# buaacyw/GaussianEditor

Hardware: AMD Instinct MI355X
Metric: train iters/sec (fwd+bwd of one 1080p view per GPU + grad all-reduce), 1M Gaussians @1080p (higher is better)
Workload: dtype f32; 1 GPU; synth-v1 1000000 Gaussians SH3 (M=16, s0=0.01), 1920x1080, ring-v1 8 views, one view per GPU (BASELINE.json configs[3] shape; configs[1] bicycle.ply is not available offline); gaussians=1000000, width=1920, height=1080, views_per_rank=1, parallelism=dp1-views, view_pipeline=False, tile_bounds=reference, fast_exp=False, grad_exchange=direct, grad_exchange_route=local, grad_rows=every row of every gradient written every iteration, num_rendered=0, visible=0, pixel_instances=0, sort_key_bits=45

## Files before the change

gaussianeditor_amd/csrc/gsr_binning.hip:

```cpp
#include <stdlib.h>

#include "gsr_kernels.h"

namespace gsr {

__device__ __forceinline__ int f2i_sat(float v) {
  if (!(v == v)) return 0;
  if (v >= 2147483648.0f) return 2147483647;
  if (v <= -2147483648.0f) return (-2147483647 - 1);
  return (int)v;
}

constexpr int RBITS = 8;
constexpr int RBINS = 1 << RBITS;

template <class K, int TH, bool WEIGHTED = false>
__global__ void __launch_bounds__(TH) sort_hist_kernel(const K* __restrict__ keys, int64_t n, int shift,
                                                                uint32_t mask, uint32_t* __restrict__ hist,
                                                                uint32_t nblocks, const uint4* __restrict__ publish_src,
                                                                uint32_t publish_count, uint32_t* __restrict__ publish_dst,
                                                                uint32_t publish_seq, const uint32_t* __restrict__ rect32) {
  __shared__ uint32_t h[RBINS];
  __shared__ uint32_t hw[WEIGHTED ? RBINS : 1];
  if (publish_dst != nullptr && blockIdx.x == nblocks) {
// ... 597 lines not shown
    constexpr int NV = (int)(sizeof(K) * RANGE_PER / sizeof(uint4));
    const uint4* __restrict__ src = reinterpret_cast<const uint4*>(tkeys + base);
    uint4 v[NV];
#pragma unroll
    for (int i = 0; i < NV; ++i) v[i] = src[i];
    __builtin_memcpy(k, v, sizeof(k));
  } else {
#pragma unroll
    for (int i = 0; i < RANGE_PER; ++i) k[i] = base + i < L ? tkeys[base + i] : (K)0;
  }
  uint32_t prev = base ? (uint32_t)tkeys[base - 1] : 0u;
#pragma unroll
  for (int i = 0; i < RANGE_PER; ++i) {
    const int64_t idx = base + i;
    if (idx >= L) break;
    const uint32_t cur = (uint32_t)k[i];
    if (idx == 0) {
      ranges[cur].x = 0;
    } else if (cur != prev) {
      ranges[prev].y = (uint32_t)idx;
      ranges[cur].x = (uint32_t)idx;
    }
    if (idx == L - 1) ranges[cur].y = (uint32_t)L;
    prev = cur;
  }
}

__global__ void __launch_bounds__(1024) tile_worklist_kernel(int T, uint2* __restrict__ ranges,
                                                            uint32_t* __restrict__ order, uint32_t* __restrict__ meta,
                                                            uint32_t* __restrict__ queues, uint32_t* __restrict__ est,
                                                            const uint32_t* __restrict__ tile_total,
                                                            uint32_t* __restrict__ tile_start, uint32_t* __restrict__ ck_table,
                                                            uint32_t n_ck_tiles) {
  constexpr int WORK_SUB = 16, NCNT = (WORK_BUCKETS + 1) * WORK_SUB, WORK_LDS_TILES = 8192;
  __shared__ uint32_t cnt[NCNT];
  __shared__ uint32_t smem[1024 / 64 + 1];
  __shared__ uint32_t s_len[WORK_LDS_TILES];
  const bool cached = T <= WORK_LDS_TILES;
  const bool split = gridDim.x == 2;
  const bool do_prefix = tile_total != nullptr && (!split || blockIdx.x == 0);
  const bool do_sort = !split || blockIdx.x == 1;
  for (int i = threadIdx.x; i < NCNT; i += 1024) cnt[i] = 0;
  if (do_prefix) {
    constexpr int PER = 8;
    uint32_t carry = 0;
    for (int base = 0; base < T; base += 1024 * PER) {
      const int i0 = base + (int)threadIdx.x * PER;
      const bool full = i0 + PER <= T;
      uint32_t v[PER], sum = 0;
      if (full) {
        const uint4 a0 = reinterpret_cast<const uint4*>(tile_total + i0)[0], a1 = reinterpret_cast<const uint4*>(tile_total + i0)[1];
        v[0] = a0.x; v[1] = a0.y; v[2] = a0.z; v[3] = a0.w; v[4] = a1.x; v[5] = a1.y; v[6] = a1.z; v[7] = a1.w;
      } else {
#pragma unroll
        for (int j = 0; j < PER; ++j) v[j] = i0 + j < T ? tile_total[i0 + j] : 0u;
      }
#pragma unroll
      for (int j = 0; j < PER; ++j) sum += v[j];
      uint32_t chunk;
      uint32_t run = carry + block_excl_scan_u32<1024>(sum, &chunk, smem);
      uint32_t st[PER];
#pragma unroll
      for (int j = 0; j < PER; ++j) {
        st[j] = run;
        run += v[j];
      }
      if (full) {
        reinterpret_cast<uint4*>(tile_start + i0)[0] = make_uint4(st[0], st[1], st[2], st[3]);
        reinterpret_cast<uint4*>(tile_start + i0)[1] = make_uint4(st[4], st[5], st[6], st[7]);
#pragma unroll
        for (int j = 0; j < PER; j += 2)
          reinterpret_cast<uint4*>(ranges + i0)[j / 2] = make_uint4(v[j] ? st[j] : 0u, v[j] ? st[j] + v[j] : 0u,
                                                                   v[j + 1] ? st[j + 1] : 0u, v[j + 1] ? st[j + 1] + v[j + 1] : 0u);
      }
#pragma unroll
      for (int j = 0; j < PER; ++j) {
        if (i0 + j < T) {
          if (!full) {
            tile_start[i0 + j] = st[j];
            ranges[i0 + j] = v[j] ? make_uint2(st[j], st[j] + v[j]) : make_uint2(0u, 0u);
          }
          if (cached) s_len[i0 + j] = v[j];
        }
      }
      carry += chunk;
    }
    if (threadIdx.x == 0) tile_start[T] = carry;
  } else if (cached && tile_total != nullptr) {
    for (int t = threadIdx.x; t < T; t += 1024) s_len[t] = tile_total[t];
  } else if (cached) {
    for (int t = threadIdx.x; t < T; t += 1024) {
      const uint2 r = ranges[t];
      s_len[t] = r.y - r.x;
    }
  }
  if (!do_sort) return;
  __syncthreads();
  auto len_of = [&](int t) -> uint32_t {
    if (cached) return s_len[t];
    if (tile_total != nullptr) return tile_total[t];
    const uint2 r = ranges[t];
    return r.y - r.x;
  };
  const uint32_t sub = threadIdx.x & (WORK_SUB - 1);
  auto bucket_of = [](uint32_t len) -> uint32_t {
    if (len == 0) return WORK_BUCKETS;
    const uint32_t c = (len + 63u) / 64u;
    return (uint32_t)(WORK_BUCKETS - 1) - min(c - 1u, (uint32_t)(WORK_BUCKETS - 1));
  };
  for (int t = threadIdx.x; t < T; t += 1024) atomicAdd(&cnt[bucket_of(len_of(t)) * WORK_SUB + sub], 1u);
  __syncthreads();
  {
    constexpr int CPT = (NCNT + 1023) / 1024;
    const int i0 = (int)threadIdx.x * CPT;
    uint32_t v[CPT], sum = 0;
#pragma unroll
    for (int j = 0; j < CPT; ++j) {
      v[j] = i0 + j < NCNT ? cnt[i0 + j] : 0u;
      sum += v[j];
    }
    uint32_t all;
    uint32_t run = block_excl_scan_u32<1024>(sum, &all, smem);
#pragma unroll
    for (int j = 0; j < CPT; ++j) {
      if (i0 + j < NCNT) cnt[i0 + j] = run;
      if (i0 + j == WORK_BUCKETS * WORK_SUB) meta[0] = run;
      run += v[j];
    }
  }
  __syncthreads();
  for (int t = threadIdx.x; t < T; t += 1024) {
    const uint32_t len = len_of(t);
    const uint32_t pos = atomicAdd(&cnt[bucket_of(len) * WORK_SUB + sub], 1u);
    order[pos] = (uint32_t)t;
    ck_table[t] = (len != 0u && pos < n_ck_tiles) ? pos : CK_NONE;
  }
  for (int i = threadIdx.x; i < 8 * T; i += 1024) est[i] = 0u;
  for (int i = threadIdx.x; i < QUEUE_KINDS * QUEUE_LINES; i += 1024) {
    queues[(size_t)i * QUEUE_STRIDE] = 0u;
    queues[(size_t)i * QUEUE_STRIDE + 1] = 0u;
  }
}

template <int BITS, int TH>
__global__ void __launch_bounds__(TH) group_hist_kernel(const uint32_t* __restrict__ keys, int64_t n,
                                                                 uint32_t* __restrict__ hist, uint32_t nblocks,
                                                                 uint32_t* __restrict__ fill_dst, int64_t fill_n) {
  constexpr int NB = 1 << BITS;
  __shared__ uint32_t h[NB];
  for (int i = threadIdx.x; i < NB; i += TH) h[i] = 0;
  (void)fill_dst;
  (void)fill_n;
  __syncthreads();
  const int64_t base = (int64_t)blockIdx.x * SORT_KPB;
  uint32_t kv[(SORT_KPB / TH)];
#pragma unroll
  for (int i = 0; i < (SORT_KPB / TH); ++i) {
    const int64_t k = base + (int64_t)i * TH + threadIdx.x;
    kv[i] = (uint32_t)keys[k < n ? k : n - 1];
  }
#pragma unroll
  for (int i = 0; i < (SORT_KPB / TH); ++i) {
    const int64_t k = base + (int64_t)i * TH + threadIdx.x;
    if (k < n) atomicAdd(&h[kv[i] & (NB - 1)], 1u);
  }
  __syncthreads();
  for (int i = threadIdx.x; i < NB; i += TH) hist[(size_t)i * nblocks + blockIdx.x] = h[i];
}

template <int BITS, int TH>
__global__ void __launch_bounds__(TH) group_scatter_kernel(const uint32_t* __restrict__ keys_in,
                                                                    const uint32_t* __restrict__ vals_in,
                                                                    uint32_t* __restrict__ keys_out,
                                                                    uint32_t* __restrict__ vals_out, int64_t n,
                                                                    const uint32_t* __restrict__ hist,
                                                                    const uint32_t* __restrict__ bin_total,
                                                                    uint32_t nblocks, uint32_t chunk,
                                                                    uint32_t* __restrict__ group_first) {
  constexpr int NB = 1 << BITS, NW = TH / 64, ITEMS = SORT_KPB / TH;
  constexpr int BT = NB < TH ? NB : TH, BPT = NB / BT;
  const bool owns = (int)threadIdx.x < BT;
  __shared__ uint16_t cnt[NW][NB];
  __shared__ uint32_t gbase[NB];
  __shared__ uint16_t lexcl[NB];
  __shared__ uint32_t smem[TH / 64 + 1];
  __shared__ uint32_t skey[SORT_KPB];
  __shared__ uint32_t sval[SORT_KPB];
  const int w = (int)(threadIdx.x >> 6), l = lane_id();
  const int64_t bbase = (int64_t)blockIdx.x * SORT_KPB;
  const int64_t wbase = bbase + (int64_t)w * (ITEMS * 64);
  uint32_t key[ITEMS], val[ITEMS];
  uint16_t rank[ITEMS];
  const uint64_t lt_mask = (1ull << l) - 1ull;
#pragma unroll
  for (int i = 0; i < ITEMS; ++i) {
    const int64_t k = wbase + (int64_t)i * 64 + l;
    const int64_t kc = k < n ? k : n - 1;
    key[i] = keys_in[kc];
    val[i] = vals_in[kc];
  }
  {
    uint32_t padded[BPT], mine[BPT], sum = 0;
#pragma unroll
    for (int j = 0; j < BPT; ++j) {
      const uint32_t d = owns ? threadIdx.x * BPT + j : 0u;
      const uint32_t tot = owns ? bin_total[d] : 0u;
      padded[j] = (tot + chunk - 1u) / chunk * chunk;
      mine[j] = owns ? hist[(size_t)d * nblocks + blockIdx.x] : 0u;
      sum += padded[j];
    }
    uint32_t tot;
    uint32_t run = block_excl_scan_u32<TH>(sum, &tot, smem);
    if (owns) {
#pragma unroll
      for (int j = 0; j < BPT; ++j) {
        gbase[threadIdx.x * BPT + j] = run + mine[j];
        if (blockIdx.x == 0) group_first[threadIdx.x * BPT + j] = run / chunk;
        run += padded[j];
      }
      if (blockIdx.x == 0 && (int)threadIdx.x == BT - 1) group_first[NB] = run / chunk;
    }
  }
  for (int i = threadIdx.x; i < NW * NB; i += TH) (&cnt[0][0])[i] = 0;
  __syncthreads();

#pragma unroll
  for (int i = 0; i < ITEMS; ++i) {
    const int64_t k = wbase + (int64_t)i * 64 + l;
    const bool valid = k < n;
    const uint32_t d = key[i] & (NB - 1);
    uint64_t m = __ballot(valid);
#pragma unroll
    for (int b = 0; b < BITS; ++b) {
      const uint64_t bb = __ballot((d >> b) & 1u);
      m &= ((d >> b) & 1u) ? bb : ~bb;
    }
    const uint32_t before = (uint32_t)__popcll(m & lt_mask);
    uint32_t old = 0;
    if (valid) old = cnt[w][d];
    if (valid && before == 0) cnt[w][d] = (uint16_t)(old + (uint32_t)__popcll(m));
    rank[i] = (uint16_t)(old + before);
  }
  __syncthreads();
  {
    uint32_t tot_d[BPT], sum = 0;
#pragma unroll
    for (int j = 0; j < BPT; ++j) {
      const uint32_t d = owns ? threadIdx.x * BPT + j : 0u;
      uint32_t run = 0;
      if (owns) {
#pragma unroll
        for (int i = 0; i < NW; ++i) {
          const uint32_t c = cnt[i][d];
          cnt[i][d] = (uint16_t)run;
          run += c;
        }
      }
      tot_d[j] = run;
      sum += run;
    }
    uint32_t tot;
    uint32_t run = block_excl_scan_u32<TH>(sum, &tot, smem);
    if (owns) {
#pragma unroll
      for (int j = 0; j < BPT; ++j) {
        lexcl[threadIdx.x * BPT + j] = (uint16_t)run;
        run += tot_d[j];
      }
    }
  }
  __syncthreads();
#pragma unroll
  for (int i = 0; i < ITEMS; ++i) {
    const int64_t k = wbase + (int64_t)i * 64 + l;
    if (k < n) {
      const uint32_t d = key[i] & (NB - 1);
      const uint32_t lp = (uint32_t)lexcl[d] + (uint32_t)cnt[w][d] + rank[i];
      skey[lp] = key[i];
      sval[lp] = val[i];
    }
  }
  __syncthreads();
  const int nvalid = (int)min((int64_t)SORT_KPB, n - bbase);
#pragma unroll
  for (int i = 0; i < ITEMS; ++i) {
    const int j = i * TH + (int)threadIdx.x;
    if (j < nvalid) {
      const uint32_t kk = skey[j], d = kk & (NB - 1);
      const uint32_t pos = gbase[d] + ((uint32_t)j - (uint32_t)lexcl[d]);
      keys_out[pos] = kk;
      vals_out[pos] = sval[j];
    }
  }
}

struct GroupArgs {
  int gx, gy, sgx;
  size_t chunks;
  uint32_t stage_cap;
  const uint32_t* gkey;
  const uint32_t* gval;
  uint16_t* chunk_cnt;
  const uint32_t* chunk_pre;
  const uint32_t* tile_start;
  uint32_t* point_list;
};

__device__ __forceinline__ void group_mask(uint32_t lr, uint32_t& lo, uint32_t& hi) {
  const uint32_t x0 = lr & 7u, x1 = (lr >> 3) & 7u, y0 = (lr >> 6) & 7u, y1 = (lr >> 9) & 7u;
  const uint32_t cols = ((2u << (x1 - x0)) - 1u) << x0;
  const uint64_t rows = ((~0ull >> (56u - 8u * (y1 - y0))) << (8u * y0)) & 0x0101010101010101ull;
  lo = (uint32_t)rows * cols;
  hi = (uint32_t)(rows >> 32) * cols;
}

struct TransposeLane {
  uint32_t keep[5], rot[5];
};
__device__ __forceinline__ TransposeLane transpose_lane_consts(int lane) {
  constexpr uint32_t LOW[5] = {0x0000ffffu, 0x00ff00ffu, 0x0f0f0f0fu, 0x33333333u, 0x55555555u};
  TransposeLane c;
#pragma unroll
  for (int i = 0; i < 5; ++i) {
    const int d = 16 >> i;
    const bool up = (lane & d) != 0;
    c.keep[i] = up ? ~LOW[i] : LOW[i];
    c.rot[i] = up ? (uint32_t)d : (uint32_t)(32 - d);
  }
  return c;
}
template <int STAGE>
__device__ __forceinline__ uint32_t transpose_partner(uint32_t x) {
  const int v = (int)x;
  if constexpr (STAGE == 0) return (uint32_t)__builtin_amdgcn_ds_swizzle(v, 0x401f);
  else if constexpr (STAGE == 1) return (uint32_t)__builtin_amdgcn_update_dpp(0, v, 0x128, 0xf, 0xf, false);
  else if constexpr (STAGE == 2) return (uint32_t)__builtin_amdgcn_ds_swizzle(v, 0x101f);
  else if constexpr (STAGE == 3) return (uint32_t)__builtin_amdgcn_update_dpp(0, v, 0x4e, 0xf, 0xf, false);
  else return (uint32_t)__builtin_amdgcn_update_dpp(0, v, 0xb1, 0xf, 0xf, false);
}
template <int STAGE>
__device__ __forceinline__ void transpose_stage(const TransposeLane& c, uint32_t& lo, uint32_t& hi) {
  const uint32_t pl = transpose_partner<STAGE>(lo), ph = transpose_partner<STAGE>(hi);
  const uint32_t rl = __builtin_amdgcn_alignbit(pl, pl, c.rot[STAGE]), rh = __builtin_amdgcn_alignbit(ph, ph, c.rot[STAGE]);
  lo = (c.keep[STAGE] & lo) | (~c.keep[STAGE] & rl);
  hi = (c.keep[STAGE] & hi) | (~c.keep[STAGE] & rh);
}
__device__ __forceinline__ void transpose_masks(const TransposeLane& c, uint32_t lo, uint32_t hi, uint32_t& wlo, uint32_t& whi) {
  {
    const auto r = __builtin_amdgcn_permlane32_swap(lo, hi, false, false);
    lo = r[0];
    hi = r[1];
  }
  transpose_stage<0>(c, lo, hi);
  transpose_stage<1>(c, lo, hi);
  transpose_stage<2>(c, lo, hi);
  transpose_stage<3>(c, lo, hi);
  transpose_stage<4>(c, lo, hi);
  wlo = lo;
  whi = hi;
}

template <bool SCATTER, int NB>
__global__ void __launch_bounds__(64) group_chunk_kernel(const GroupArgs a) {
  extern __shared__ __align__(8) unsigned char stage_raw[];
  uint2* const stage = reinterpret_cast<uint2*>(stage_raw);
  const size_t c = (size_t)(blockIdx.x & 7u) * (gridDim.x >> 3) + (blockIdx.x >> 3);
  if (c >= a.chunks) return;
  const int lane = (int)threadIdx.x;
  const size_t base = c * (size_t)(64 * NB);
  uint32_t key[NB], idx[NB];
#pragma unroll
  for (int b = 0; b < NB; ++b) {
    key[b] = a.gkey[base + (size_t)b * 64 + lane];
    idx[b] = SCATTER ? a.gval[base + (size_t)b * 64 + lane] : 0u;
  }
  const uint32_t first = (uint32_t)__builtin_amdgcn_readfirstlane((int)key[0]);
  if (first == GROUP_PAD) return;
  const TransposeLane tc = transpose_lane_consts(lane);
  const uint32_t cap = a.stage_cap;
  uint32_t cnt = 0, g = 0, staged = 0;
  if (SCATTER) {
    const uint32_t s = first & 0xffffu;
    const uint32_t tx = ((s % (uint32_t)a.sgx) << GROUP_SHIFT) + (uint32_t)(lane & 7);
    const uint32_t ty = ((s / (uint32_t)a.sgx) << GROUP_SHIFT) + (uint32_t)(lane >> 3);
    const bool tile_ok = tx < (uint32_t)a.gx && ty < (uint32_t)a.gy;
    g = tile_ok ? a.tile_start[ty * (uint32_t)a.gx + tx] + a.chunk_pre[c * GROUP_TILES + lane] : 0u;
  }
  auto flush = [&]() {
    __syncthreads();
    for (uint32_t e = (uint32_t)lane; e < staged; e += 64u) {
      const uint2 x = stage[e];
      a.point_list[x.y] = x.x;
    }
    __syncthreads();
    staged = 0;
  };
#pragma unroll
  for (int b = 0; b < NB; ++b) {
    const bool valid = key[b] != GROUP_PAD;
    if (b > 0 && __ballot(valid) == 0ull) break;
    uint32_t lo = 0u, hi = 0u;
    if (valid) group_mask(key[b] >> 16, lo, hi);
    uint32_t wlo, whi;
    transpose_masks(tc, lo, hi, wlo, whi);
    if (!SCATTER) {
      cnt += (uint32_t)__popc(wlo) + (uint32_t)__popc(whi);
    } else {
      const uint32_t nl = (uint32_t)__popc(wlo), nh = (uint32_t)__popc(whi);
      const uint32_t tot_l = (uint32_t)__builtin_amdgcn_readlane((int)wave_incl_scan_dpp(nl), 63);
      const uint32_t tot_h = (uint32_t)__builtin_amdgcn_readlane((int)wave_incl_scan_dpp(nh), 63);
      const int nparts = tot_l + tot_h <= cap ? 1 : (max(tot_l, tot_h) <= cap ? 2 : 4);
      for (int part = 0; part < nparts; ++part) {
        uint32_t wa = wlo, wb = whi;
        if (nparts == 2) {
          wa = part == 0 ? wlo : 0u;
          wb = part == 0 ? 0u : whi;
        } else if (nparts == 4) {
          const uint32_t m = 0xffffu << (16 * (part & 1));
          wa = part < 2 ? (wlo & m) : 0u;
          wb = part < 2 ? 0u : (whi & m);
        }
        const uint32_t na = (uint32_t)__popc(wa), np = na + (uint32_t)__popc(wb);
        const uint32_t incl = wave_incl_scan_dpp(np);
        const uint32_t total = (uint32_t)__builtin_amdgcn_readlane((int)incl, 63);
        if (staged + total > cap) flush();
        uint32_t curA = staged + incl - np, curB = curA + na, gA = g, gB = g + na;
        while (__ballot((wa | wb) != 0u) != 0ull) {
          const bool va = wa != 0u, vb = wb != 0u;
          const int ja = va ? __builtin_ctz(wa) : 0, jb = vb ? 32 + __builtin_ctz(wb) : 0;
          const uint32_t xa = (uint32_t)__shfl((int)idx[b], ja, 64), xb = (uint32_t)__shfl((int)idx[b], jb, 64);
          stage[va ? curA : cap] = make_uint2(xa, gA);
          stage[vb ? curB : cap] = make_uint2(xb, gB);
          curA += va ? 1u : 0u;
          gA += va ? 1u : 0u;
          curB += vb ? 1u : 0u;
          gB += vb ? 1u : 0u;
          wa &= wa - 1u;
          wb &= wb - 1u;
        }
        staged += total;
        g += np;
      }
    }
  }
  if (SCATTER) flush();
  if (!SCATTER) a.chunk_cnt[c * GROUP_TILES + lane] = (uint16_t)cnt;
}

constexpr int COLSCAN_WAVES = 16, COLSCAN_REG = 16;
__global__ void __launch_bounds__(COLSCAN_WAVES * 64) group_colscan_kernel(int gx, int gy, int sgx,
                                                                          const uint32_t* __restrict__ group_first,
                                                                          const uint16_t* __restrict__ chunk_cnt,
                                                                          uint32_t* __restrict__ chunk_pre,
                                                                          uint32_t* __restrict__ tile_total) {
  __shared__ uint32_t slab[COLSCAN_WAVES][GROUP_TILES];
  const uint32_t s = blockIdx.x;
  const int w = (int)(threadIdx.x >> 6), lane = lane_id();
  const uint32_t first = group_first[s], n = group_first[s + 1] - first;
  const uint32_t per = (n + COLSCAN_WAVES - 1) / COLSCAN_WAVES;
  const uint32_t r0 = min(n, (uint32_t)w * per), r1 = min(n, r0 + per);
  const uint16_t* __restrict__ src = chunk_cnt + (size_t)(first + r0) * GROUP_TILES + lane;
  uint32_t* __restrict__ out = chunk_pre + (size_t)(first + r0) * GROUP_TILES + lane;
  const uint32_t rows = r1 - r0;
  auto load_rows = [&](uint32_t first_row, uint32_t (&v)[COLSCAN_REG]) {
    const uint32_t last = rows - 1u;
    uint32_t raw[COLSCAN_REG];
#pragma unroll
    for (int i = 0; i < COLSCAN_REG; ++i) raw[i] = (uint32_t)src[(size_t)min(first_row + (uint32_t)i, last) * GROUP_TILES];
#pragma unroll
    for (int i = 0; i < COLSCAN_REG; ++i) v[i] = first_row + (uint32_t)i < rows ? raw[i] : 0u;
  };
  uint32_t v0[COLSCAN_REG];
  uint32_t sum = 0;
#pragma unroll
  for (int i = 0; i < COLSCAN_REG; ++i) v0[i] = 0u;
  if (rows != 0u) {
    load_rows(0u, v0);
#pragma unroll
    for (int i = 0; i < COLSCAN_REG; ++i) sum += v0[i];
    for (uint32_t r = COLSCAN_REG; r < rows; r += COLSCAN_REG) {
      uint32_t v[COLSCAN_REG];
      load_rows(r, v);
#pragma unroll
      for (int i = 0; i < COLSCAN_REG; ++i) sum += v[i];
    }
  }
  slab[w][lane] = sum;
  __syncthreads();
  uint32_t run = 0, total = 0;
#pragma unroll
  for (int i = 0; i < COLSCAN_WAVES; ++i) {
    const uint32_t x = slab[i][lane];
    run += i < w ? x : 0u;
    total += x;
  }
#pragma unroll
  for (int i = 0; i < COLSCAN_REG; ++i) {
    if ((uint32_t)i < rows) out[(size_t)i * GROUP_TILES] = run;
    run += v0[i];
  }
  for (uint32_t r = COLSCAN_REG; r < rows; r += COLSCAN_REG) {
    uint32_t v[COLSCAN_REG];
    load_rows(r, v);
#pragma unroll
    for (int i = 0; i < COLSCAN_REG; ++i) {
      if (r + (uint32_t)i < rows) out[(size_t)(r + (uint32_t)i) * GROUP_TILES] = run;
      run += v[i];
    }
  }
  if (w == 0) {
    const uint32_t tx = ((s % (uint32_t)sgx) << GROUP_SHIFT) + (uint32_t)(lane & 7);
    const uint32_t ty = ((s / (uint32_t)sgx) << GROUP_SHIFT) + (uint32_t)(lane >> 3);
    if (tx < (uint32_t)gx && ty < (uint32_t)gy) tile_total[ty * (uint32_t)gx + tx] = total;
  }
}

template <bool SCATTER>
static void launch_chunks(hipStream_t s, const Binning& b, const GroupArgs& a) {
  const dim3 grid((unsigned)((b.chunks + 7) / 8 * 8)), block(64);
  const size_t lds = SCATTER ? sizeof(uint2) * ((size_t)a.stage_cap + 1) : 0;
  switch (b.chunk / 64) {
    case 1: hipLaunchKernelGGL((group_chunk_kernel<SCATTER, 1>), grid, block, lds, s, a); break;
    case 2: hipLaunchKernelGGL((group_chunk_kernel<SCATTER, 2>), grid, block, lds, s, a); break;
    case 4: hipLaunchKernelGGL((group_chunk_kernel<SCATTER, 4>), grid, block, lds, s, a); break;
    default: hipLaunchKernelGGL((group_chunk_kernel<SCATTER, 8>), grid, block, lds, s, a); break;
  }
}

static int64_t checkpoint_state_words(const Image& im);
template <int BITS>
static void launch_grouped(hipStream_t s, int P, int64_t R, int gx, int gy, const Geom& g, const Binning& b, const Image& im) {
  const int nbg = (P + GAUSS_BLOCK - 1) / GAUSS_BLOCK;
  const int64_t padded = b.chunks * (int64_t)b.chunk;
  const int fill_blocks = 512;
  hipLaunchKernelGGL(emit_groups_kernel, dim3(nbg + fill_blocks), dim3(GAUSS_BLOCK), 0, s, P, b.sgx, g, b.gkey[0], b.gval[0], nbg,
                     b.gkey[1], padded, reinterpret_cast<uint4*>(im.ck_work), checkpoint_state_words(im) / 4);
  const bool wide = b.sort_blocks <= SORT_WIDE_MAX_BLOCKS;
  if (wide)
    hipLaunchKernelGGL((group_hist_kernel<BITS, 1024>), dim3(b.sort_blocks), dim3(1024), 0, s, (const uint32_t*)b.gkey[0], b.G,
                       b.ghist, b.sort_blocks, b.gkey[1], padded);
  else
    hipLaunchKernelGGL((group_hist_kernel<BITS, SORT_THREADS>), dim3(b.sort_blocks), dim3(SORT_THREADS), 0, s,
                       (const uint32_t*)b.gkey[0], b.G, b.ghist, b.sort_blocks, b.gkey[1], padded);
  hipLaunchKernelGGL(sort_scan_kernel, dim3(1 << BITS), dim3(SORT_THREADS), 0, s, b.ghist, b.gbin_total, b.sort_blocks);
  if (wide)
    hipLaunchKernelGGL((group_scatter_kernel<BITS, 1024>), dim3(b.sort_blocks), dim3(1024), 0, s, (const uint32_t*)b.gkey[0],
                       (const uint32_t*)b.gval[0], b.gkey[1], b.gval[1], b.G, (const uint32_t*)b.ghist,
                       (const uint32_t*)b.gbin_total, b.sort_blocks, (uint32_t)b.chunk, b.group_first);
  else
    hipLaunchKernelGGL((group_scatter_kernel<BITS, SORT_THREADS>), dim3(b.sort_blocks), dim3(SORT_THREADS), 0, s,
                       (const uint32_t*)b.gkey[0], (const uint32_t*)b.gval[0], b.gkey[1], b.gval[1], b.G, (const uint32_t*)b.ghist,
                       (const uint32_t*)b.gbin_total, b.sort_blocks, (uint32_t)b.chunk, b.group_first);
  GroupArgs a;
  a.gx = gx; a.gy = gy; a.sgx = b.sgx; a.chunks = (size_t)b.chunks;
  a.stage_cap = (R / b.G + 1) * (int64_t)b.chunk <= 820 ? 1024u : 2048u;
  a.gkey = b.gkey[1]; a.gval = b.gval[1];
  a.chunk_cnt = b.chunk_cnt; a.chunk_pre = b.chunk_pre; a.tile_start = b.tile_start; a.point_list = b.point_list;
  launch_chunks<false>(s, b, a);
  hipLaunchKernelGGL(group_colscan_kernel, dim3(b.groups), dim3(COLSCAN_WAVES * 64), 0, s, gx, gy, b.sgx,
                     (const uint32_t*)b.group_first, (const uint16_t*)b.chunk_cnt, b.chunk_pre, b.tile_total);
  hipLaunchKernelGGL(tile_worklist_kernel, dim3(2), dim3(1024), 0, s, gx * gy, im.ranges, im.work_order, im.work_meta,
                     im.queue_heads, im.work_est, (const uint32_t*)b.tile_total, b.tile_start, im.ck_table,
                     (uint32_t)ck_tiles((size_t)gx * gy));
  launch_chunks<true>(s, b, a);
}

static int64_t checkpoint_state_words(const Image& im) {
  return (int64_t)((reinterpret_cast<const char*>(im.ck_pool) - reinterpret_cast<const char*>(im.ck_work)) / 4);
}

hipError_t launch_binning(hipStream_t s, int P, int64_t R, int W, int H, const Geom& g, const Binning& b, const Image& im) {
  const int gx = (W + TILE - 1) / TILE, gy = (H + TILE - 1) / TILE;
  if (R <= 0 || b.legacy) {
    hipError_t e = hipMemsetAsync(im.ck_work, 0, sizeof(uint32_t) * (size_t)checkpoint_state_words(im), s);
    if (e != hipSuccess) return e;
  }
  if (R <= 0) {
    hipError_t e = hipMemsetAsync(im.ranges, 0, sizeof(uint2) * (size_t)gx * gy, s);
    if (e != hipSuccess) return e;
    hipLaunchKernelGGL(tile_worklist_kernel, dim3(1), dim3(1024), 0, s, gx * gy, im.ranges, im.work_order, im.work_meta,
                       im.queue_heads, im.work_est, (const uint32_t*)nullptr, (uint32_t*)nullptr, im.ck_table,
                       (uint32_t)ck_tiles((size_t)gx * gy));
    return hipGetLastError();
  }
  if (!b.legacy) {
    if (b.group_bits == 8) launch_grouped<8>(s, P, R, gx, gy, g, b, im);
    else launch_grouped<11>(s, P, R, gx, gy, g, b, im);
    return hipGetLastError();
  }
  const int nbg = (P + GAUSS_BLOCK - 1) / GAUSS_BLOCK;
  const dim3 ge(max(nbg, (gx * gy + GAUSS_BLOCK - 1) / GAUSS_BLOCK)), gr((unsigned)((R + 256 * RANGE_PER - 1) / (256 * RANGE_PER)));
  if (b.key_bytes == 2) {
    uint16_t* const tk[2] = {(uint16_t*)b.tkey[0], (uint16_t*)b.tkey[1]};
    hipLaunchKernelGGL(emit_keys_kernel<uint16_t>, ge, dim3(GAUSS_BLOCK), 0, s, P, gx, gx * gy, g, tk[0], b.vals[0], im.ranges);
    radix_sort_pairs<uint16_t>(s, tk, b.vals, R, b.passes, b.digit_bits, b.hist, b.bin_total, false);
    hipLaunchKernelGGL(tile_ranges_kernel<uint16_t>, gr, dim3(256), 0, s, R, (const uint16_t*)tk[b.final_buf], im.ranges);
  } else {
    uint32_t* const tk[2] = {(uint32_t*)b.tkey[0], (uint32_t*)b.tkey[1]};
    hipLaunchKernelGGL(emit_keys_kernel<uint32_t>, ge, dim3(GAUSS_BLOCK), 0, s, P, gx, gx * gy, g, tk[0], b.vals[0], im.ranges);
    radix_sort_pairs<uint32_t>(s, tk, b.vals, R, b.passes, b.digit_bits, b.hist, b.bin_total, false);
    hipLaunchKernelGGL(tile_ranges_kernel<uint32_t>, gr, dim3(256), 0, s, R, (const uint32_t*)tk[b.final_buf], im.ranges);
  }
  hipLaunchKernelGGL(tile_worklist_kernel, dim3(1), dim3(1024), 0, s, gx * gy, im.ranges, im.work_order, im.work_meta,
                     im.queue_heads, im.work_est, (const uint32_t*)nullptr, (uint32_t*)nullptr, im.ck_table,
                     (uint32_t)ck_tiles((size_t)gx * gy));
  return hipGetLastError();
}

template <class K>
__global__ void __launch_bounds__(256) export_keys_kernel(int64_t R, const K* __restrict__ tkeys,
                                                         const uint32_t* __restrict__ vals, const float4* __restrict__ rec1,
                                                         uint64_t* __restrict__ keys) {
  const int64_t i = (int64_t)blockIdx.x * 256 + threadIdx.x;
  if (i >= R) return;
  keys[i] = ((uint64_t)tkeys[i] << 32) | (uint64_t)__float_as_uint(rec1[vals[i]].z);
}
__global__ void __launch_bounds__(256) export_keys_grouped_kernel(int64_t R, uint32_t T, const uint32_t* __restrict__ tile_start,
                                                                 const uint32_t* __restrict__ vals,
                                                                 const float4* __restrict__ rec1, uint64_t* __restrict__ keys) {
  const int64_t i = (int64_t)blockIdx.x * 256 + threadIdx.x;
  if (i >= R) return;
  uint32_t lo = 0, hi = T;
  while (hi - lo > 1u) {
    const uint32_t mid = (lo + hi) >> 1;
    if ((int64_t)tile_start[mid] <= i) lo = mid; else hi = mid;
  }
  keys[i] = ((uint64_t)lo << 32) | (uint64_t)__float_as_uint(rec1[vals[i]].z);
}
hipError_t launch_export_keys(hipStream_t s, int64_t R, int W, int H, const Binning& b, const Geom& g, uint64_t* keys) {
  const dim3 grid((unsigned)((R + 255) / 256));
  if (!b.legacy) {
    const uint32_t T = (uint32_t)(((W + TILE - 1) / TILE) * ((H + TILE - 1) / TILE));
    hipLaunchKernelGGL(export_keys_grouped_kernel, grid, dim3(256), 0, s, R, T, (const uint32_t*)b.tile_start,
                       (const uint32_t*)b.point_list, g.rec1, keys);
  } else if (b.key_bytes == 2) {
    hipLaunchKernelGGL(export_keys_kernel<uint16_t>, grid, dim3(256), 0, s, R, (const uint16_t*)b.tkey[b.final_buf],
                       b.vals[b.final_buf], g.rec1, keys);
  } else {
    hipLaunchKernelGGL(export_keys_kernel<uint32_t>, grid, dim3(256), 0, s, R, (const uint32_t*)b.tkey[b.final_buf],
                       b.vals[b.final_buf], g.rec1, keys);
  }
  return hipGetLastError();
}

}
```

Baseline: 1822 view-iters/s.

## Fold per-chunk counts into 16-row block scans before column scan

The count pass now runs 16 chunks per block and writes inclusive prefix sums within each 16-row block, split at group boundaries, using LDS. The column scan then reads only the last row of each block, so it scans far fewer rows. The scatter pass rebuilds each chunk's prefix from the block-level prefix plus the in-block inclusive count of the previous row. This replaces a long serial per-group column scan with a two-level scan, at the cost of extra LDS work and more complex offset logic that could be wrong at group or block edges.

After: 1825 view-iters/s, median of 2. About the same (+0.1%).

```diff
diff --git a/gaussianeditor_amd/csrc/gsr_binning.hip b/gaussianeditor_amd/csrc/gsr_binning.hip
--- a/gaussianeditor_amd/csrc/gsr_binning.hip
+++ b/gaussianeditor_amd/csrc/gsr_binning.hip
@@ -923,6 +923,7 @@
   const uint32_t* gval;
   uint16_t* chunk_cnt;
   const uint32_t* chunk_pre;
+  const uint32_t* group_first;
   const uint32_t* tile_start;
   uint32_t* point_list;
 };
@@ -981,14 +982,18 @@
   whi = hi;
 }
 
+constexpr int COUNT_ROWS = 16;
 template <bool SCATTER, int NB>
-__global__ void __launch_bounds__(64) group_chunk_kernel(const GroupArgs a) {
+__global__ void __launch_bounds__(SCATTER ? 64 : COUNT_ROWS * 64) group_chunk_kernel(const GroupArgs a) {
   extern __shared__ __align__(8) unsigned char stage_raw[];
   uint2* const stage = reinterpret_cast<uint2*>(stage_raw);
-  const size_t c = (size_t)(blockIdx.x & 7u) * (gridDim.x >> 3) + (blockIdx.x >> 3);
-  if (c >= a.chunks) return;
-  const int lane = (int)threadIdx.x;
-  const size_t base = c * (size_t)(64 * NB);
+  uint32_t (*const s_cnt)[GROUP_TILES] = reinterpret_cast<uint32_t (*)[GROUP_TILES]>(stage_raw);
+  uint32_t* const s_gid = reinterpret_cast<uint32_t*>(stage_raw) + COUNT_ROWS * GROUP_TILES;
+  const int lane = lane_id(), w = (int)(threadIdx.x >> 6);
+  const size_t c = SCATTER ? (size_t)(blockIdx.x & 7u) * (gridDim.x >> 3) + (blockIdx.x >> 3)
+                           : (size_t)blockIdx.x * COUNT_ROWS + (size_t)w;
+  if (SCATTER && c >= a.chunks) return;
+  const size_t base = (SCATTER ? c : min(c, a.chunks - 1)) * (size_t)(64 * NB);
   uint32_t key[NB], idx[NB];
 #pragma unroll
   for (int b = 0; b < NB; ++b) {
@@ -996,7 +1001,8 @@
     idx[b] = SCATTER ? a.gval[base + (size_t)b * 64 + lane] : 0u;
   }
   const uint32_t first = (uint32_t)__builtin_amdgcn_readfirstlane((int)key[0]);
-  if (first == GROUP_PAD) return;
+  if (SCATTER && first == GROUP_PAD) return;
+  const bool live = SCATTER || (c < a.chunks && first != GROUP_PAD);
   const TransposeLane tc = transpose_lane_consts(lane);
   const uint32_t cap = a.stage_cap;
   uint32_t cnt = 0, g = 0, staged = 0;
@@ -1005,7 +1011,12 @@
     const uint32_t tx = ((s % (uint32_t)a.sgx) << GROUP_SHIFT) + (uint32_t)(lane & 7);
     const uint32_t ty = ((s / (uint32_t)a.sgx) << GROUP_SHIFT) + (uint32_t)(lane >> 3);
     const bool tile_ok = tx < (uint32_t)a.gx && ty < (uint32_t)a.gy;
-    g = tile_ok ? a.tile_start[ty * (uint32_t)a.gx + tx] + a.chunk_pre[c * GROUP_TILES + lane] : 0u;
+    const uint32_t gf = a.group_first[s];
+    const size_t c0 = c & ~(size_t)(COUNT_ROWS - 1);
+    const uint32_t above = (uint32_t)a.chunk_cnt[(c != 0 ? c - 1 : 0) * GROUP_TILES + lane];
+    const uint32_t ahead = a.chunk_pre[(c / COUNT_ROWS) * GROUP_TILES + lane];
+    const uint32_t pre = ((size_t)gf < c0 ? ahead : 0u) + ((c == c0 || c == (size_t)gf) ? 0u : above);
+    g = tile_ok ? a.tile_start[ty * (uint32_t)a.gx + tx] + pre : 0u;
   }
   auto flush = [&]() {
     __syncthreads();
@@ -1018,8 +1029,8 @@
   };
 #pragma unroll
   for (int b = 0; b < NB; ++b) {
-    const bool valid = key[b] != GROUP_PAD;
-    if (b > 0 && __ballot(valid) == 0ull) break;
+    const bool valid = live && key[b] != GROUP_PAD;
+    if ((b > 0 || !SCATTER) && __ballot(valid) == 0ull) break;
     uint32_t lo = 0u, hi = 0u;
     if (valid) group_mask(key[b] >> 16, lo, hi);
     uint32_t wlo, whi;
@@ -1065,7 +1076,16 @@
     }
   }
   if (SCATTER) flush();
-  if (!SCATTER) a.chunk_cnt[c * GROUP_TILES + lane] = (uint16_t)cnt;
+  if (!SCATTER) {
+    const uint32_t gid = live ? (first & 0xffffu) : GROUP_PAD;
+    s_cnt[w][lane] = cnt;
+    if (lane == 0) s_gid[w] = gid;
+    __syncthreads();
+    uint32_t sum = 0;
+#pragma unroll
+    for (int i = 0; i < COUNT_ROWS; ++i) sum += (i <= w && s_gid[i] == gid) ? s_cnt[i][lane] : 0u;
+    if (live) a.chunk_cnt[c * GROUP_TILES + lane] = (uint16_t)sum;
+  }
 }
 
 constexpr int COLSCAN_WAVES = 16, COLSCAN_REG = 16;
@@ -1077,17 +1097,22 @@
   __shared__ uint32_t slab[COLSCAN_WAVES][GROUP_TILES];
   const uint32_t s = blockIdx.x;
   const int w = (int)(threadIdx.x >> 6), lane = lane_id();
-  const uint32_t first = group_first[s], n = group_first[s + 1] - first;
+  const uint32_t first = group_first[s], nrows = group_first[s + 1] - first;
+  const uint32_t last_row = first + nrows - 1u, b0 = first / COUNT_ROWS;
+  const uint32_t n = nrows != 0u ? last_row / COUNT_ROWS - b0 + 1u : 0u;
   const uint32_t per = (n + COLSCAN_WAVES - 1) / COLSCAN_WAVES;
   const uint32_t r0 = min(n, (uint32_t)w * per), r1 = min(n, r0 + per);
-  const uint16_t* __restrict__ src = chunk_cnt + (size_t)(first + r0) * GROUP_TILES + lane;
-  uint32_t* __restrict__ out = chunk_pre + (size_t)(first + r0) * GROUP_TILES + lane;
+  const uint16_t* __restrict__ src = chunk_cnt + lane;
+  uint32_t* __restrict__ out = chunk_pre + (size_t)(b0 + r0) * GROUP_TILES + lane;
   const uint32_t rows = r1 - r0;
   auto load_rows = [&](uint32_t first_row, uint32_t (&v)[COLSCAN_REG]) {
     const uint32_t last = rows - 1u;
     uint32_t raw[COLSCAN_REG];
 #pragma unroll
-    for (int i = 0; i < COLSCAN_REG; ++i) raw[i] = (uint32_t)src[(size_t)min(first_row + (uint32_t)i, last) * GROUP_TILES];
+    for (int i = 0; i < COLSCAN_REG; ++i) {
+      const uint32_t blk = b0 + r0 + min(first_row + (uint32_t)i, last);
+      raw[i] = (uint32_t)src[(size_t)min(blk * COUNT_ROWS + (COUNT_ROWS - 1), last_row) * GROUP_TILES];
+    }
 #pragma unroll
     for (int i = 0; i < COLSCAN_REG; ++i) v[i] = first_row + (uint32_t)i < rows ? raw[i] : 0u;
   };
@@ -1117,7 +1142,7 @@
   }
 #pragma unroll
   for (int i = 0; i < COLSCAN_REG; ++i) {
-    if ((uint32_t)i < rows) out[(size_t)i * GROUP_TILES] = run;
+    if ((uint32_t)i < rows && r0 + (uint32_t)i != 0u) out[(size_t)i * GROUP_TILES] = run;
     run += v0[i];
   }
   for (uint32_t r = COLSCAN_REG; r < rows; r += COLSCAN_REG) {
@@ -1138,8 +1163,10 @@
 
 template <bool SCATTER>
 static void launch_chunks(hipStream_t s, const Binning& b, const GroupArgs& a) {
-  const dim3 grid((unsigned)((b.chunks + 7) / 8 * 8)), block(64);
-  const size_t lds = SCATTER ? sizeof(uint2) * ((size_t)a.stage_cap + 1) : 0;
+  const dim3 grid(SCATTER ? (unsigned)((b.chunks + 7) / 8 * 8) : (unsigned)((b.chunks + COUNT_ROWS - 1) / COUNT_ROWS));
+  const dim3 block(SCATTER ? 64 : COUNT_ROWS * 64);
+  const size_t lds = SCATTER ? sizeof(uint2) * ((size_t)a.stage_cap + 1)
+                             : sizeof(uint32_t) * (size_t)(COUNT_ROWS * GROUP_TILES + COUNT_ROWS);
   switch (b.chunk / 64) {
     case 1: hipLaunchKernelGGL((group_chunk_kernel<SCATTER, 1>), grid, block, lds, s, a); break;
     case 2: hipLaunchKernelGGL((group_chunk_kernel<SCATTER, 2>), grid, block, lds, s, a); break;
@@ -1176,7 +1203,8 @@
   a.gx = gx; a.gy = gy; a.sgx = b.sgx; a.chunks = (size_t)b.chunks;
   a.stage_cap = (R / b.G + 1) * (int64_t)b.chunk <= 820 ? 1024u : 2048u;
   a.gkey = b.gkey[1]; a.gval = b.gval[1];
-  a.chunk_cnt = b.chunk_cnt; a.chunk_pre = b.chunk_pre; a.tile_start = b.tile_start; a.point_list = b.point_list;
+  a.chunk_cnt = b.chunk_cnt; a.chunk_pre = b.chunk_pre; a.group_first = b.group_first; a.tile_start = b.tile_start;
+  a.point_list = b.point_list;
   launch_chunks<false>(s, b, a);
   hipLaunchKernelGGL(group_colscan_kernel, dim3(b.groups), dim3(COLSCAN_WAVES * 64), 0, s, gx, gy, b.sgx,
                      (const uint32_t*)b.group_first, (const uint16_t*)b.chunk_cnt, b.chunk_pre, b.tile_total);
```
